# eikehmueller/mlmcpathintegral

Hardware: AMD Instinct MI355X
Metric: lattice-site-updates/sec (higher is better)
Workload: dtype f64

## Files before the change

### mlmcpathintegral_amd/csrc/schwinger_perm.hpp

```cpp
#pragma once
#include "lattice_sweep.hpp"

namespace mlmcpi {

#ifdef MLMCPI_STAMPS
__device__ unsigned long long g_stamps[16 * 65536];
#define MLMCPI_STAMP(k)                                                                                            \
  do {                                                                                                             \
    if (threadIdx.x == 0 && blockIdx.y * gridDim.x + blockIdx.x < 65536)                                           \
      g_stamps[(blockIdx.y * gridDim.x + blockIdx.x) * 16 + (k)] = __builtin_amdgcn_s_memrealtime();               \
  } while (0)
#define MLMCPI_STAMP_WHERE()                                                                                       \
  do {                                                                                                             \
    if (threadIdx.x == 0 && blockIdx.y * gridDim.x + blockIdx.x < 65536)                                           \
      g_stamps[(blockIdx.y * gridDim.x + blockIdx.x) * 16 + 15] =                                                  \
          ((unsigned long long)__builtin_amdgcn_s_getreg((20 ) | (0 << 6) | (31 << 11)) << 32) |         \
          __builtin_amdgcn_s_getreg((4 ) | (0 << 6) | (31 << 11));                                        \
  } while (0)
#else
#define MLMCPI_STAMP(k) do { } while (0)
#define MLMCPI_STAMP_WHERE() do { } while (0)
#endif

#ifndef MLMCPI_PERM_U
#define MLMCPI_PERM_U 0
#endif

template <class PG>
struct PermPlane {
  static constexpr int kRow = PG::kPitch * 8, kStep = kRow + 8;
  static constexpr uint32_t QB = (uint32_t)PG::kQRows * kRow;
  static_assert(kStep == (int)PG::kStep * 8, "the stride of a stream");
  uint32_t K;
  __device__ __forceinline__ explicit PermPlane(uint32_t K_) : K(K_) {}
  __device__ __forceinline__ bool has_col(uint32_t C) const { return (C & 1u) ? C <= PG::col_last(K, 1) : C >= PG::col_first(K, 0) && C <= PG::col_last(K, 0); }
  __device__ __forceinline__ bool has_row(uint32_t R) const { return (R & 1u) ? R <= PG::row_last(K, 1) : R >= PG::row_first(K, 0) && R <= PG::row_last(K, 0); }
  __device__ __forceinline__ uint32_t col(uint32_t C) const { return (C & 1u) ? QB + PG::col_u(K, C) * 8u : PG::col_u(K, C) * 8u; }
  __device__ __forceinline__ uint32_t row(uint32_t R) const { return (R & 1u) ? 2u * QB + PG::row_v(K, R) * (uint32_t)kRow : PG::row_v(K, R) * (uint32_t)kRow; }
};

struct PermBuildPos {
  uint32_t c, r, rend, row_off, gj;
  uint32_t cb;
  const double2 *src;
  uint32_t col;
  bool active, owns;
};
template <int NT, class PP>
__device__ __forceinline__ PermBuildPos perm_build_pos(const PP &P, const double2 *__restrict__ src, uint32_t Mt, uint32_t Mx, uint32_t gi0,
                                                       uint32_t gj0, uint32_t W, uint32_t rows) {
  PermBuildPos q;
  const uint32_t wave = __builtin_amdgcn_readfirstlane(threadIdx.x / kWave), lane = threadIdx.x % kWave;
  const uint32_t nwc = W > 63 ? 2 : 1;
  const uint32_t groups = (NT / kWave) >> (nwc - 1);
  const uint32_t g = wave >> (nwc - 1), cw = wave & (nwc - 1);
  static_assert(((NT / kWave) & (NT / kWave - 1)) == 0, "waves per workgroup: a power of two (shifts for divisions)");
  const uint32_t rpg = groups == 4 ? (rows + 3) >> 2 : groups == 8 ? (rows + 7) >> 3 : (rows + groups - 1) / groups;
  q.c = 63 * cw + lane;
  q.r = __builtin_amdgcn_readfirstlane(g * rpg);
  q.rend = __builtin_amdgcn_readfirstlane(g < groups ? min(rows, q.r + rpg) : 0);
  q.active = q.r < q.rend;
  q.owns = lane < 63 && q.c < W && P.has_col(q.c);
  q.cb = P.col(q.c);
  q.src = src;
  q.col = wrap_add(gi0, min(q.c, W), Mt);
  q.gj = __builtin_amdgcn_readfirstlane(wrap_add(gj0, q.r, Mx));
  q.row_off = q.gj * Mt;
  return q;
}
template <int U>
__device__ __forceinline__ void perm_rows_load(PermBuildPos &q, uint32_t Mt, uint32_t Mx, bool first, double2 &cur, double2 (&nxt)[U]) {
  if (!q.active) return;
  if (first) cur = (q.src + q.row_off)[q.col];
#pragma unroll
  for (int u = 0; u < U; ++u) {
    q.gj = q.gj + 1 == Mx ? 0 : q.gj + 1;
    q.row_off = q.gj == 0 ? 0 : q.row_off + Mt;
    if (q.r + u < q.rend) nxt[u] = (q.src + q.row_off)[q.col];
  }
}
template <int U, class PP>
__device__ __forceinline__ void perm_rows_store(PermBuildPos &q, const PP &P, double *plane, double2 &cur, const double2 (&nxt)[U]) {
  if (!q.active) return;
  char *const pb = reinterpret_cast<char *>(plane) + q.cb;
#pragma unroll
  for (int u = 0; u < U; ++u)
    if (q.r + u < q.rend) {
      const double right = wave_rotate_down(cur.y);
      if (q.owns && P.has_row(q.r + u)) *reinterpret_cast<double *>(pb + P.row(q.r + u)) = ((cur.x + right) - nxt[u].x) - cur.y;
      cur = nxt[u];
    }
  q.r += U;
}
template <int NT, int U, bool ONCE, class PP>
__device__ __forceinline__ void perm_build_rows(const PP &P, double *plane, const double2 *__restrict__ src, uint32_t Mt, uint32_t Mx,
                                                uint32_t gi0, uint32_t gj0, uint32_t W, uint32_t rows) {
  PermBuildPos q = perm_build_pos<NT>(P, src, Mt, Mx, gi0, gj0, W, rows);
  double2 cur = make_double2(0., 0.);
  if (ONCE) {
    double2 nxt[U];
    perm_rows_load<U>(q, Mt, Mx, true, cur, nxt);
    perm_rows_store<U>(q, P, plane, cur, nxt);
    return;
  }
  bool first = true;
  while (__builtin_amdgcn_readfirstlane(q.r) < __builtin_amdgcn_readfirstlane(q.rend)) {
    double2 nxt[U];
    perm_rows_load<U>(q, Mt, Mx, first, cur, nxt);
    perm_rows_store<U>(q, P, plane, cur, nxt);
    first = false;
  }
}

template <int NT, int RING, int TH = 64>
struct PermTasks {
  using PG = PermGeom<NT, RING, TH>;
  static constexpr int OW = PG::OW, HR = PG::HR, H2 = HR / 2, NW = NT / kWave, NS = PG::NV;
  static constexpr int NWK = NW / 2, Q = H2 / NWK, R = H2 % NWK;
  static constexpr int XC = OW - 64;
  static constexpr int L0 = XC * H2, L1 = (XC / 2) * HR;
  static constexpr int NL0 = (L0 + 63) / 64, NL1 = (L1 + 63) / 64;
  static_assert(NW % 2 == 0 && NS == Q + (R > 0 ? 1 : 0), "slots per thread: the longer block");
  static_assert(XC == 0 || (R > 0 && NL0 <= NWK - R && NL1 <= NWK - R), "the left-over wave-tasks fit the free last slots of their kind");
  uint32_t wave, lane, c_mu0, c_mu1, r_lo;
  uint32_t j, m0, len;
  bool kind;
  __device__ PermTasks() {
    wave = __builtin_amdgcn_readfirstlane(threadIdx.x / kWave);
    lane = threadIdx.x % kWave;
    c_mu0 = lane < 32 ? 2 * lane : 2 * (lane - 32) + 1;
    c_mu1 = 2 * (lane & 31u);
    r_lo = lane >> 5;
    kind = wave >= (uint32_t)NWK;
    j = kind ? wave - (uint32_t)NWK : wave;
    m0 = j * (uint32_t)Q + min(j, (uint32_t)R);
    len = (uint32_t)Q + (j < (uint32_t)R ? 1u : 0u);
  }
  template <class F>
  __device__ __forceinline__ void by_kind(F &&f) const {
    if (kind) f(std::true_type{}); else f(std::false_type{});
  }
  __device__ __forceinline__ bool in_block(int k) const { return k < Q || (uint32_t)k < len; }
  template <bool MU1>
  __device__ __forceinline__ bool task(int k, uint32_t &r, uint32_t &c) const {
    if (main_task<MU1>(k, r, c)) return true;
    return XC > 0 && k == NS - 1 && left_task<MU1>(r, c);
  }
  template <bool MU1>
  __device__ __forceinline__ bool main_task(int k, uint32_t &r, uint32_t &c) const {
    r = 0; c = 0;
    if (!in_block(k)) return false;
    const uint32_t m = m0 + (uint32_t)k;
    r = MU1 ? 2 * m + r_lo : 2 * m;
    c = MU1 ? c_mu1 : c_mu0;
    return true;
  }
  template <bool MU1>
  __device__ __forceinline__ bool left_task(uint32_t &r, uint32_t &c) const {
    r = 0; c = 0;
    if (XC > 0 && !in_block(NS - 1)) {
      const uint32_t jl = j - (uint32_t)R;
      if (!MU1 && jl < (uint32_t)NL0) {
        const uint32_t L = 64 * jl + lane;
        r = 2 * (L / (XC ? XC : 1));
        c = 64 + L % (XC ? XC : 1);
        return L < (uint32_t)L0;
      }
      if (MU1 && jl < (uint32_t)NL1) {
        const uint32_t L = 64 * jl + lane;
        r = L / (XC > 1 ? XC / 2 : 1);
        c = 64 + 2 * (L % (XC > 1 ? XC / 2 : 1));
        return L < (uint32_t)L1;
      }
    }
    return false;
  }
};

template <int STEP>
__device__ __forceinline__ void perm_gather5(uint32_t pa, uint32_t px, uint32_t px2, double &S, double &X, double &X2) {
  double a0 = lds_read_f64<0>(pa), x0 = lds_read_f64<0>(px), y0 = lds_read_f64<0>(px2);
  double a1 = lds_read_f64<STEP>(pa), x1 = lds_read_f64<STEP>(px), y1 = lds_read_f64<STEP>(px2);
  double a2 = lds_read_f64<2 * STEP>(pa), x2 = lds_read_f64<2 * STEP>(px), y2 = lds_read_f64<2 * STEP>(px2);
  double a3 = lds_read_f64<3 * STEP>(pa), x3 = lds_read_f64<3 * STEP>(px), y3 = lds_read_f64<3 * STEP>(px2);
  double a4 = lds_read_f64<4 * STEP>(pa), x4 = lds_read_f64<4 * STEP>(px), y4 = lds_read_f64<4 * STEP>(px2);
  asm volatile("s_waitcnt lgkmcnt(0)"
               : "+v"(a0), "+v"(x0), "+v"(y0), "+v"(a1), "+v"(x1), "+v"(y1), "+v"(a2), "+v"(x2), "+v"(y2), "+v"(a3), "+v"(x3), "+v"(y3),
                 "+v"(a4), "+v"(x4), "+v"(y4)
               :
               : "memory");
  S += a0; X += x0; X2 += y0;
  S += a1; X += x1; X2 += y1;
  S += a2; X += x2; X2 += y2;
  S += a3; X += x3; X2 += y3;
  S += a4; X += x4; X2 += y4;
}
__device__ __forceinline__ void perm_gather1(uint32_t pa, uint32_t px, uint32_t px2, double &S, double &X, double &X2) {
  double a0 = lds_read_f64<0>(pa), x0 = lds_read_f64<0>(px), y0 = lds_read_f64<0>(px2);
  asm volatile("s_waitcnt lgkmcnt(0)" : "+v"(a0), "+v"(x0), "+v"(y0) : : "memory");
  S += a0; X += x0; X2 += y0;
}
template <int STEP>
__device__ __forceinline__ void perm_gather5(uint32_t pa, uint32_t px2, double &S, double &X2) {
  double a0 = lds_read_f64<0>(pa), y0 = lds_read_f64<0>(px2);
  double a1 = lds_read_f64<STEP>(pa), y1 = lds_read_f64<STEP>(px2);
  double a2 = lds_read_f64<2 * STEP>(pa), y2 = lds_read_f64<2 * STEP>(px2);
  double a3 = lds_read_f64<3 * STEP>(pa), y3 = lds_read_f64<3 * STEP>(px2);
  double a4 = lds_read_f64<4 * STEP>(pa), y4 = lds_read_f64<4 * STEP>(px2);
  asm volatile("s_waitcnt lgkmcnt(0)"
               : "+v"(a0), "+v"(y0), "+v"(a1), "+v"(y1), "+v"(a2), "+v"(y2), "+v"(a3), "+v"(y3), "+v"(a4), "+v"(y4)
               :
               : "memory");
  S += a0; X2 += y0;
  S += a1; X2 += y1;
  S += a2; X2 += y2;
  S += a3; X2 += y3;
  S += a4; X2 += y4;
}
__device__ __forceinline__ void perm_gather1(uint32_t pa, uint32_t px2, double &S, double &X2) {
  double a0 = lds_read_f64<0>(pa), y0 = lds_read_f64<0>(px2);
  asm volatile("s_waitcnt lgkmcnt(0)" : "+v"(a0), "+v"(y0) : : "memory");
  S += a0; X2 += y0;
}

template <int NT, int RING, int TH = 64>
__device__ __forceinline__ void perm_sweeps(double *plane, const double2 *__restrict__ src, uint32_t Mt, uint32_t Mx, uint32_t i0,
                                            uint32_t j0, uint32_t K, double2 (&res)[2][PermGeom<NT, RING, TH>::NV]) {
  using PG = PermGeom<NT, RING, TH>;
  using PP = PermPlane<PG>;
  constexpr int HR = PG::HR, NV = PG::NV;
  constexpr int kGroups = NT / kWave / 2;
  constexpr int U = MLMCPI_PERM_U ? MLMCPI_PERM_U : (2 * HR + 4 * (int)kPermMaxK + kGroups - 1) / kGroups;
  const uint32_t W = PG::width(K), rows = PG::rows(K), H = RING + 2 * K;
  const PP P(K);
  auto back = [](uint32_t x, uint32_t h, uint32_t n) { return h <= n ? (x >= h ? x - h : x + n - h) : (x + n - h % n) % n; };
  const uint32_t gi0 = back(i0, H, Mt), gj0 = back(j0, H, Mx);
  const uint32_t oi0 = back(i0, RING, Mt), oj0 = back(j0, RING, Mx);
  using PT = PermTasks<NT, RING, TH>;
  const PT tasks;
  const char *const src_b = reinterpret_cast<const char *>(src);
  const bool small_lattice = Mx < (uint32_t)(2 * HR + 2) || Mt < (uint32_t)(PG::OW + 2);
  auto load_theta_of = [&](int h, double2 (&th)[NV], auto small, auto kind) {
    constexpr bool MU1 = decltype(kind)::value;
#pragma unroll
    for (int k = 0; k < NV; ++k) {
      uint32_t r, c;
      if (!tasks.template task<MU1>(k, r, c)) continue;
      uint32_t gr = oj0 + r + h * HR, gc = oi0 + c;
      gr = min(gr, gr - Mx);
      gc = min(gc, gc - Mt);
      if ((bool)small) {
        gr = min(gr, gr - Mx); gr = min(gr, gr - Mx);
        gc = min(gc, gc - Mt); gc = min(gc, gc - Mt);
      }
      const uint32_t o = (gr * Mt + gc) * 16u;
      if (!MU1) {
        const uint32_t o2 = gr + 1 == Mx ? o - gr * Mt * 16u : o + Mt * 16u;
        th[k] = make_double2(*reinterpret_cast<const double *>(src_b + o), *reinterpret_cast<const double *>(src_b + o2));
      } else {
        const uint32_t o2 = gc + 1 == Mt ? o - gc * 16u : o + 16u;
        th[k] = make_double2(*reinterpret_cast<const double *>(src_b + o + 8u), *reinterpret_cast<const double *>(src_b + o2 + 8u));
      }
    }
  };
  auto load_theta = [&](int h, double2 (&th)[NV], auto kind) {
    if (small_lattice) load_theta_of(h, th, std::true_type{}, kind); else load_theta_of(h, th, std::false_type{}, kind);
  };
  auto gather = [&](int h, double2 (&d)[NV], auto kind) {
    constexpr bool MU1 = decltype(kind)::value;
    const uint32_t lds0 = (uint32_t)(uintptr_t)plane;
    double Xnext = 0.0;
    auto one = [&](int k, uint32_t r, uint32_t c, auto chained_t) {
      constexpr bool chained = decltype(chained_t)::value;
      const uint32_t ro = r + (uint32_t)(h * HR), cq = c >> 1, rq = ro >> 1;
      uint32_t a, x, x2;
      if (!MU1) {
        const uint32_t cb = (c & 1u) ? PP::QB + ((uint32_t)(PG::OW / 2 - 1) - cq) * 8u : cq * 8u;
        x = cb + rq * (uint32_t)PP::kRow;
        x2 = x + (uint32_t)PP::kRow;
        a = cb + 2u * PP::QB + ((uint32_t)(HR - 1) - rq) * (uint32_t)PP::kRow;
      } else {
        const uint32_t rb = (ro & 1u) ? 2u * PP::QB + ((uint32_t)(HR - 1) - rq) * (uint32_t)PP::kRow : (rq + 1u) * (uint32_t)PP::kRow;
        x = rb + cq * 8u;
        x2 = x + 8u;
        a = rb + PP::QB + ((uint32_t)(PG::OW / 2) - cq) * 8u;
      }
      uint32_t pa = lds0 + a, px = lds0 + x, px2 = lds0 + x2;
      double S = 0.0, X = 0.0, X2 = 0.0;
      uint32_t s = 0;
      if (chained) {
        X = Xnext;
        for (; s + 5 <= K; s += 5) {
          perm_gather5<PP::kStep>(pa, px2, S, X2);
          pa += 5 * PP::kStep;
          px2 += 5 * PP::kStep;
        }
        for (; s < K; ++s) {
          perm_gather1(pa, px2, S, X2);
          pa += PP::kStep;
          px2 += PP::kStep;
        }
      } else {
        for (; s + 5 <= K; s += 5) {
          perm_gather5<PP::kStep>(pa, px, px2, S, X, X2);
          pa += 5 * PP::kStep;
          px += 5 * PP::kStep;
          px2 += 5 * PP::kStep;
        }
        for (; s < K; ++s) {
          perm_gather1(pa, px, px2, S, X, X2);
          pa += PP::kStep;
          px += PP::kStep;
          px2 += PP::kStep;
        }
      }
      Xnext = X2;
      double2 dk = MU1 ? make_double2(X - S, X2 - S) : make_double2(S - X, S - X2);
      asm volatile("" : "+v"(dk.x), "+v"(dk.y));
      d[k] = dk;
    };
    uint32_t r, c;
    if (PT::XC > 0)
      if (tasks.template left_task<MU1>(r, c)) one(NV - 1, r, c, std::false_type{});
#pragma unroll
    for (int k = 0; k < NV; ++k) {
      if (!tasks.template main_task<MU1>(k, r, c)) continue;
      if (!MU1 && k > 0) one(k, r, c, std::true_type{}); else one(k, r, c, std::false_type{});
    }
  };
  auto finish = [&](const double2 (&th)[NV], double2 (&d)[NV], auto kind) {
#pragma unroll
    for (int k = 0; k < NV; ++k) {
      uint32_t r, c;
      if (tasks.template task<decltype(kind)::value>(k, r, c)) d[k] = make_double2(mod_2pi_fast(th[k].x + d[k].x), mod_2pi_fast(th[k].y + d[k].y));
    }
  };

  perm_build_rows<NT, U, MLMCPI_PERM_U == 0>(P, plane, src, Mt, Mx, gi0, gj0, W, rows);
  double2 th[NV];
  tasks.by_kind([&](auto kind) { load_theta(0, th, kind); });
  __syncthreads();
  MLMCPI_STAMP(1);
  tasks.by_kind([&](auto kind) {
    gather(0, res[0], kind);
    finish(th, res[0], kind);
    MLMCPI_STAMP(2);
    load_theta(1, th, kind);
    gather(1, res[1], kind);
    finish(th, res[1], kind);
  });
}

template <int NT, int RING, int TH = 64>
__device__ __forceinline__ void perm_store_image(double *th0, double *th1, const double2 (&res)[2][PermGeom<NT, RING, TH>::NV]) {
  using PG = PermGeom<NT, RING, TH>;
  constexpr int OW = PG::OW, HR = PG::HR, NV = PG::NV;
  const PermTasks<NT, RING, TH> tasks;
  tasks.by_kind([&](auto kind) {
    constexpr bool MU1 = decltype(kind)::value;
#pragma unroll
    for (int h = 0; h < 2; ++h)
#pragma unroll
      for (int k = 0; k < NV; ++k) {
        uint32_t r, c;
        if (!tasks.template task<MU1>(k, r, c)) continue;
        const uint32_t o = (r + h * HR) * OW + c;
        if (!MU1) {
          th0[o] = res[h][k].x;
          th0[o + OW] = res[h][k].y;
        } else {
          th1[o] = res[h][k].x;
          th1[o + 1] = res[h][k].y;
        }
      }
  });
}

}
```

Measured before the change: 1028 billion.

## Share mu=1 neighbour sums across lanes via DPP instead of extra LDS gathers

For the mu=1 link kind, each lane now gathers only its own X sum from LDS. The neighbouring X2 sum is taken from the adjacent lane with a wave rotate plus DPP row-shift edge patching, and the boundary values come from one extra 'edge' gather done only in the first slot. This is meant to cut LDS read traffic in the gather loop for mu=1, which previously read three streams per site. In exchange it adds cross-lane DPP shuffles, a per-slot switch, and layout assumptions about lane-to-site mapping that are intricate and could be wrong at row edges.

```diff
diff --git a/mlmcpathintegral_amd/csrc/schwinger_perm.hpp b/mlmcpathintegral_amd/csrc/schwinger_perm.hpp
--- a/mlmcpathintegral_amd/csrc/schwinger_perm.hpp
+++ b/mlmcpathintegral_amd/csrc/schwinger_perm.hpp
@@ -222,6 +222,29 @@
   asm volatile("s_waitcnt lgkmcnt(0)" : "+v"(a0), "+v"(y0) : : "memory");
   S += a0; X2 += y0;
 }
+template <int KS>
+__device__ __forceinline__ int perm_edge_patch(int rot, int e) {
+  static_assert(KS >= 0 && KS < 16, "a slot of the block per lane of a DPP row");
+  if (KS > 0) e = __builtin_amdgcn_update_dpp(0, e, 0x100 + (KS > 0 ? KS : 1) , 0xF, 0xF, true);
+  return __builtin_amdgcn_update_dpp(rot, e, 0x11F , 0xA , 0xF, false);
+}
+template <int KS>
+__device__ __forceinline__ double perm_next_pair(double X, double E) {
+  const double rot = wave_rotate_down(X);
+  return __hiloint2double(perm_edge_patch<KS>(__double2hiint(rot), __double2hiint(E)), perm_edge_patch<KS>(__double2loint(rot), __double2loint(E)));
+}
+__device__ __forceinline__ double perm_next_pair(double X, double E, int k) {
+  switch (k) {
+    case 0: return perm_next_pair<0>(X, E);
+    case 1: return perm_next_pair<1>(X, E);
+    case 2: return perm_next_pair<2>(X, E);
+    case 3: return perm_next_pair<3>(X, E);
+    case 4: return perm_next_pair<4>(X, E);
+    case 5: return perm_next_pair<5>(X, E);
+    case 6: return perm_next_pair<6>(X, E);
+    default: return perm_next_pair<7>(X, E);
+  }
+}
 
 template <int NT, int RING, int TH = 64>
 __device__ __forceinline__ void perm_sweeps(double *plane, const double2 *__restrict__ src, uint32_t Mt, uint32_t Mx, uint32_t i0,
@@ -266,12 +289,19 @@
   auto load_theta = [&](int h, double2 (&th)[NV], auto kind) {
     if (small_lattice) load_theta_of(h, th, std::true_type{}, kind); else load_theta_of(h, th, std::false_type{}, kind);
   };
+  constexpr int kThree = 0, kChained = 1, kShared = 2, kEdge = 3;
   auto gather = [&](int h, double2 (&d)[NV], auto kind) {
     constexpr bool MU1 = decltype(kind)::value;
     const uint32_t lds0 = (uint32_t)(uintptr_t)plane;
     double Xnext = 0.0;
-    auto one = [&](int k, uint32_t r, uint32_t c, auto chained_t) {
-      constexpr bool chained = decltype(chained_t)::value;
+    double E = 0.0;
+    uint32_t edge = 0;
+    auto row_mu1 = [](uint32_t ro) {
+      const uint32_t rq = ro >> 1;
+      return (ro & 1u) ? 2u * PP::QB + ((uint32_t)(HR - 1) - rq) * (uint32_t)PP::kRow : (rq + 1u) * (uint32_t)PP::kRow;
+    };
+    auto one = [&](int k, uint32_t r, uint32_t c, auto mode_t) {
+      constexpr int mode = decltype(mode_t)::value;
       const uint32_t ro = r + (uint32_t)(h * HR), cq = c >> 1, rq = ro >> 1;
       uint32_t a, x, x2;
       if (!MU1) {
@@ -280,7 +310,7 @@
         x2 = x + (uint32_t)PP::kRow;
         a = cb + 2u * PP::QB + ((uint32_t)(HR - 1) - rq) * (uint32_t)PP::kRow;
       } else {
-        const uint32_t rb = (ro & 1u) ? 2u * PP::QB + ((uint32_t)(HR - 1) - rq) * (uint32_t)PP::kRow : (rq + 1u) * (uint32_t)PP::kRow;
+        const uint32_t rb = row_mu1(ro);
         x = rb + cq * 8u;
         x2 = x + 8u;
         a = rb + PP::QB + ((uint32_t)(PG::OW / 2) - cq) * 8u;
@@ -288,7 +318,7 @@
       uint32_t pa = lds0 + a, px = lds0 + x, px2 = lds0 + x2;
       double S = 0.0, X = 0.0, X2 = 0.0;
       uint32_t s = 0;
-      if (chained) {
+      if (mode == kChained) {
         X = Xnext;
         for (; s + 5 <= K; s += 5) {
           perm_gather5<PP::kStep>(pa, px2, S, X2);
@@ -300,6 +330,33 @@
           pa += PP::kStep;
           px2 += PP::kStep;
         }
+      } else if (mode == kShared) {
+        for (; s + 5 <= K; s += 5) {
+          perm_gather5<PP::kStep>(pa, px, S, X);
+          pa += 5 * PP::kStep;
+          px += 5 * PP::kStep;
+        }
+        for (; s < K; ++s) {
+          perm_gather1(pa, px, S, X);
+          pa += PP::kStep;
+          px += PP::kStep;
+        }
+        X2 = perm_next_pair(X, E, k);
+      } else if (mode == kEdge) {
+        uint32_t pe = lds0 + edge;
+        for (; s + 5 <= K; s += 5) {
+          perm_gather5<PP::kStep>(pa, px, pe, S, X, E);
+          pa += 5 * PP::kStep;
+          px += 5 * PP::kStep;
+          pe += 5 * PP::kStep;
+        }
+        for (; s < K; ++s) {
+          perm_gather1(pa, px, pe, S, X, E);
+          pa += PP::kStep;
+          px += PP::kStep;
+          pe += PP::kStep;
+        }
+        X2 = perm_next_pair(X, E, k);
       } else {
         for (; s + 5 <= K; s += 5) {
           perm_gather5<PP::kStep>(pa, px, px2, S, X, X2);
@@ -321,11 +378,19 @@
     };
     uint32_t r, c;
     if (PT::XC > 0)
-      if (tasks.template left_task<MU1>(r, c)) one(NV - 1, r, c, std::false_type{});
+      if (tasks.template left_task<MU1>(r, c)) one(NV - 1, r, c, std::integral_constant<int, kThree>{});
+    if (MU1) {
+      static_assert(NV <= 8, "perm_next_pair: a case per slot");
+      const uint32_t i = tasks.lane & 15u, on = (tasks.lane & 16u) && i < tasks.len;
+      edge = row_mu1(2u * tasks.m0 + (on ? 2u * i + (tasks.lane >> 5) : 0u) + (uint32_t)(h * HR)) + 32u * 8u;
+    }
 #pragma unroll
     for (int k = 0; k < NV; ++k) {
       if (!tasks.template main_task<MU1>(k, r, c)) continue;
-      if (!MU1 && k > 0) one(k, r, c, std::true_type{}); else one(k, r, c, std::false_type{});
+      if (MU1 && k > 0) one(k, r, c, std::integral_constant<int, kShared>{});
+      else if (MU1) one(k, r, c, std::integral_constant<int, kEdge>{});
+      else if (k > 0) one(k, r, c, std::integral_constant<int, kChained>{});
+      else one(k, r, c, std::integral_constant<int, kThree>{});
     }
   };
   auto finish = [&](const double2 (&th)[NV], double2 (&d)[NV], auto kind) {
```

Result: no change. 1036 billion (median of 6 runs) (+0.8%).
